# EasyVision-Ton/VMG

Measured on AMD Instinct MI355X. Metric: LR-frames/s (train: forward+loss+backward+AdamW), VMG-REDS-few_levels 4x SR, higher is better.
Workload: dtype bf16; 1 GPU; VMG-REDS-few_levels train step, per-GPU batch 4x7x3x64x64 -> 4x SR (BASELINE configs[1]); global_batch=4, frames_per_clip=7, parallelism=dp1, launch=eager, recompute_chains=False, fp8_chains=False

## Files before the change

include/vmg_hip.h:

```cpp
#ifndef VMG_HIP_H
#define VMG_HIP_H

#include <stdint.h>

#ifdef __cplusplus
extern "C" {
#endif

#define VMG_F32 0
#define VMG_BF16 1

#define VMG_ACT_NONE 0
#define VMG_ACT_RELU 1
#define VMG_ACT_LRELU 2
#define VMG_ACT_GELU 3

#define VMG_CONV_GENERAL 0
#define VMG_CONV_KSPLIT 2
#define VMG_CONV_WS 3
#define VMG_CONV_LINEAR_WRES 4
#define VMG_CONV_WSTAT 6

const char* vmg_last_error(void);
int vmg_version(void);
// ... 234 lines not shown
int64_t vmg_win3d_attn_bwd_ws_bytes(int B, int D, int H, int W, int heads, int wt);
int vmg_win3d_attn_bwd(int dtype, const void* q, const void* kv, const float* bq, const float* bkv, const float* table, const void* out,
                       const float* lse, const void* d_out, void* dq, void* dkv, float* dtable, float* dbq, float* dbkv, void* ws, int B, int D, int H, int W,
                       int C, int heads, int wt, int sd, int sh, int sw, void* stream);
int vmg_win3d_variant(int variant);

int vmg_maxpool_fwd(int dtype, const void* x, void* y, unsigned char* idx, int N, int H, int W, int C, int f, void* stream);
int vmg_maxpool_bwd(int dtype, const void* dy, const unsigned char* idx, void* dx, int N, int H, int W, int C, int f, void* stream);

int vmg_se_mlp_fwd(const float* m, const float* w1, const float* b1, const float* w2, const float* b2, float* pre, float* out, int G, int C,
                   int Hd, int Co, int act1, int mode, void* stream);
int vmg_se_mlp_bwd(const float* dout, const float* out, const float* m, const float* pre, const float* w1, const float* w2, float* dm,
                   float* dw1, float* db1, float* dw2, float* db2, float* ws, int G, int C, int Hd, int Co, int act1, int mode, float dm_scale,
                   int accumulate, void* stream);

int vmg_avgpool2_nhwc(int dtype, const void* x, void* y, int n, int h, int w, int c, void* stream);
int vmg_upsample2x_ac_fwd(const float* x, float* y, int n, int h, int w, int c, float scale, void* stream);
int vmg_upsample2x_ac_bwd(const float* dy, float* dx, int n, int h, int w, int c, float scale, void* stream);
int vmg_spy_operand_fwd(int dtype, const void* ref, const void* warped, const float* up, void* out, int64_t npix, void* stream);
int vmg_spy_operand_bwd(int dtype, const void* dx8, void* dwarped, float* dup, int64_t npix, void* stream);
int vmg_spy_flow_add(int dtype, const float* up, const void* res, float* out, int64_t n, void* stream);
int vmg_spy_prep(int dtype, const float* img, const float* mean, const float* stdv, void* out, int64_t n, int h, int w, void* stream);
typedef struct vmg_spy_module_desc {
  int N, H, W;
  const void* x;
  const void* packed[5];
  const float* bias[5];
  void* y[4];
  void* out;
  void* dpre[4];
// ... 95 lines not shown
```

vmg_amd/csrc/tab_ops.hip:

```cpp
#include "common.h"

namespace {

template <typename T>
struct V16 {
  static constexpr int N = 16 / sizeof(T);
  T v[N];
};

template <typename T, int VN>
__global__ __launch_bounds__(256) void group_reduce_kernel(const T* __restrict__ a, const T* __restrict__ b, const T* __restrict__ c3,
                                                           float* __restrict__ out, int G, long long R, int C, int mode, float scale,
                                                           int chunks) {
  struct alignas(sizeof(T) * VN) Vec { T v[VN]; };
  __shared__ float red[VN * 256];
  const int g = blockIdx.x / chunks, ck = blockIdx.x - g * chunks;
  const int tpr = C / VN;
  const int rpb = 256 / tpr;
  const int roff = threadIdx.x / tpr, cp = threadIdx.x - roff * tpr;
  const long long r0 = R * ck / chunks, r1 = R * (ck + 1) / chunks;
  float s[VN];
#pragma unroll
  for (int e = 0; e < VN; ++e) s[e] = 0.f;
  if (roff < rpb) {
// ... 492 lines not shown
  } else if (i < n1 + n2) {
    const int e = i - n1, o = e / Hd, j = e - o * Hd;
    for (int g = 0; g < G; ++g) s += dz2[(long long)g * Co + o] * se_act(pre[g * Hd + j], act1);
    dw2[e] = accumulate ? dw2[e] + s : s;
  } else if (i < n1 + n2 + Hd) {
    const int j = i - n1 - n2;
    for (int g = 0; g < G; ++g) s += dz1[g * Hd + j];
    db1[j] = accumulate ? db1[j] + s : s;
  } else if (i < n1 + n2 + Hd + Co) {
    const int o = i - n1 - n2 - Hd;
    for (int g = 0; g < G; ++g) s += dz2[(long long)g * Co + o];
    db2[o] = accumulate ? db2[o] + s : s;
  }
}

}

extern "C" int vmg_se_mlp_fwd(const float* m, const float* w1, const float* b1, const float* w2, const float* b2, float* pre, float* out, int G,
                              int C, int Hd, int Co, int act1, int mode, void* stream) {
  VMG_CHECK(m && w1 && w2 && pre && out && G > 0 && C > 0 && Hd > 0 && Co > 0, "se_mlp_fwd: bad arguments");
  VMG_CHECK((act1 == 1 || act1 == 3) && (mode == 0 || (mode == 1 && Co % 3 == 0)), "se_mlp_fwd: act1 is ReLU (1) or GELU (3); mode 1 needs Co = 3 * channels");
  VMG_CHECK((C + Hd) * 4 <= 64 * 1024, "se_mlp_fwd: C + Hd too large");
  hipLaunchKernelGGL(se_mlp_fwd_kernel, dim3(G), dim3(1024), (C + Hd) * 4, (hipStream_t)stream, m, w1, b1, w2, b2, pre, out, C, Hd, Co, act1, mode);
  VMG_LAUNCH_CHECK();
  return 0;
}

extern "C" int vmg_se_mlp_bwd(const float* dout, const float* out, const float* m, const float* pre, const float* w1, const float* w2, float* dm,
                              float* dw1, float* db1, float* dw2, float* db2, float* ws, int G, int C, int Hd, int Co, int act1, int mode,
                              float dm_scale, int accumulate, void* stream) {
// ... 84 lines not shown
  const int chunks = gr_chunks(G, R);
  VMG_CHECK((int64_t)G * chunks * C * 3 * (int64_t)sizeof(float) <= ws_bytes, "group_reduce3: workspace too small (vmg_group_reduce_ws_bytes)");
  hipStream_t st = (hipStream_t)stream;
  if (dtype == VMG_BF16)
    hipLaunchKernelGGL((group_reduce3_kernel<bf16, 8>), dim3(G * chunks), dim3(256), 0, st, (const bf16*)a, (const bf16*)b0, (const bf16*)b1,
                       (const bf16*)b2, ws, G, (long long)R, C, scale, chunks);
  else
    hipLaunchKernelGGL((group_reduce3_kernel<float, 4>), dim3(G * chunks), dim3(256), 0, st, (const float*)a, (const float*)b0, (const float*)b1,
                       (const float*)b2, ws, G, (long long)R, C, scale, chunks);
  VMG_LAUNCH_CHECK();
  hipLaunchKernelGGL(group_reduce_final_kernel, dim3(G * cdiv(3 * C, 16)), dim3(256), 0, st, (const float*)ws, out, G, chunks, 3 * C, scale);
  VMG_LAUNCH_CHECK();
  return 0;
}

extern "C" int vmg_tab_elementwise(int dtype, int op, const void* p0, const void* p1, const void* p2, const float* coef, const float* add,
                                   float s, void* o0, void* o1, void* o2, int64_t rows, int64_t R, int C, void* stream) {
  VMG_CHECK(dtype == VMG_F32 || dtype == VMG_BF16, "tab_elementwise: bad dtype");
  VMG_CHECK(op >= 0 && op <= 9 && p0 && o0 && rows > 0 && R > 0 && rows % R == 0 && C > 0, "tab_elementwise: bad arguments");
  const int vn = dtype == VMG_BF16 ? 8 : 4;
  VMG_CHECK(C % vn == 0, "tab_elementwise: C must be a multiple of %d", vn);
  static const unsigned char uses[10] = { 1 | 4,       4 | 8 | 16,  1 | 2 | 4,       4 | 8 | 16 | 32,
                                          1,         1 | 2 | 16,  4 | 8,         4,
                                          1 | 2 | 4,  1 | 2 | 4 | 16};
  const void* const ptrs[6] = {p1, p2, coef, add, o1, o2};
  static const char* const names[6] = {"p1", "p2", "coef", "add", "o1", "o2"};
  VMG_CHECK((((uintptr_t)p0 | (uintptr_t)o0) % 16) == 0, "tab_elementwise: pointers must be 16-byte aligned");
  for (int i = 0; i < 6; ++i) {
    const bool used = (uses[op] >> i) & 1;
    VMG_CHECK(!used || ptrs[i], "tab_elementwise: op %d needs %s", op, names[i]);
// ... 52 lines not shown
```

vmg_amd/functional.py:

```python
from __future__ import annotations

import contextlib
from typing import List, Optional, Sequence

import torch

from . import hip
from . import kernels as K
from .hip import HipError
from .wgrad import DEFERRED, _wgrad_entries, _wgrad_now, flush_deferred_wgrads, recorded, set_wgrad_mode

class _Fn(torch.autograd.Function):

    @classmethod
    def apply(cls, *args):
        return super(torch.autograd.Function, cls).apply(*args)


def _pad_to(n: int, m: int = 8) -> int:
    return (n + m - 1) // m * m


def choose_tiling(M: int, cout: int, ks: int, dtype: torch.dtype, src_ch: Optional[Sequence[int]] = None, pixel_shuffle: bool = False):
    if USE_WS and src_ch is not None and not pixel_shuffle:
# ... 10 lines not shown
        if cout == 288 and src_ch[0] == 144:
            return 5, 1, hip.CONV_LINEAR_WRES
        if cout == 144 and src_ch[0] == 288:
            return 3, 1, hip.CONV_LINEAR_WRES
    if dtype == torch.bfloat16 and ks == 3 and not pixel_shuffle and M >= (1 << 18) and src_ch is not None and len(src_ch) == 1 and \
            src_ch[0] <= 64 and src_ch[0] % 8 == 0 and cout in (16, 48, 64):
        return cout // 16, 1, hip.CONV_WSTAT
    if dtype == torch.bfloat16 and ks == 3 and not pixel_shuffle and M >= (1 << 20) and src_ch is not None and len(src_ch) == 1 and \
            (cout <= 16 or src_ch[0] <= 16):
        return None, 2, hip.CONV_GENERAL
    return None, 1, hip.CONV_GENERAL


USE_WS = True
GROUPED_DENSE = True

class _PlanState:

    def __init__(self):
        self.plan, self.stamp, self.wkey, self.ents, self.packs = K.PackPlan(), -1, None, [], []


def _from_param(ent) -> bool:
    pw, weight = ent[1], ent[2]
    return pw.call is not None and pw.call[0] == weight.data_ptr()


class _PackCache:

    def __init__(self):
# ... 817 lines not shown
        axis, chunk, Cp, shape = ctx.cfg
        return K.morph_tokens_gather(g.contiguous(), axis, chunk, Cp, Cp), None, None, None, None


def morph_linear(x: torch.Tensor, weight: torch.Tensor, bias: Optional[torch.Tensor], axis: str, chunk: int, Cp: int) -> torch.Tensor:
    if K.morph_fused_ok(x, chunk, Cp):
        return _MorphLinear.apply(x, weight, bias, axis, chunk, Cp)
    tok = _MorphGather.apply(x, axis, chunk, Cp)
    if tok.shape[-1] != Cp:
        padded, tok = tok, tok[:, :Cp]
        tok._vmg_padded = padded
    t = linear(tok, weight, bias, act=hip.ACT_RELU, alpha=1.0 / Cp)
    return _MorphScatter.apply(t, axis, chunk, Cp, tuple(x.shape))


class _ChannelAttention(_Fn):

    @staticmethod
    def forward(ctx, r, x, w1, b1, w2, b2, s):
        r, x = r.contiguous(), x.contiguous()
        N, C = r.shape[0], r.shape[-1]
        R = r.numel() // (N * C)
        m = K.group_reduce(r, N, scale=1.0 / R)
        pre, g = K.se_mlp_forward(m, w1.flatten(1), b1, w2.flatten(1), b2, hip.ACT_RELU, 0)
        out = K.tab_elementwise(K.OP_CA_FWD, r, x, coef=g, s=s, G=N)
        ctx.s, ctx.R = s, R
        ctx.save_for_backward(r, g, m, pre, w1, w2)
        DEFERRED.claim(ctx, w1, b1, w2, b2)
        return out

    @staticmethod
    def backward(ctx, dy):
        r, g, m, pre, w1, w2 = ctx.saved_tensors
        s, R = ctx.s, ctx.R
        dy = dy.contiguous()
        N = r.shape[0]
        dg = K.group_reduce(dy, N, b=r, mode=1, scale=s)
        dm, dw1, db1, dw2, db2 = K.se_mlp_backward(dg, g, m, pre, w1.flatten(1), w2.flatten(1), hip.ACT_RELU, 0, 1.0 / R, into=DEFERRED.into(ctx))
        d_r, d_x = K.tab_elementwise(K.OP_CA_BWD, dy, coef=g, add=dm, s=s, G=N, nout=2)
        DEFERRED.done(ctx)
        if ctx.direct:
            return d_r, d_x, None, None, None, None, None
        return (d_r, d_x, dw1.reshape(w1.shape), db1, dw2.reshape(w2.shape), db2, None)


def channel_attention_residual(r, x, w1, b1, w2, b2, out_scale: float):
    return _ChannelAttention.apply(r, x, w1, b1, w2, b2, float(out_scale))

class _ResidualDropPath(_Fn):

    @staticmethod
    def forward(ctx, res, y, g, gb=None):
        out = K.tab_elementwise(K.OP_CA_FWD, y.contiguous(), res.contiguous(), coef=g, s=1.0, G=g.shape[0])
# ... 66 lines not shown
            mask.div_(keep)
        g = (mask * scale).expand(B, C).contiguous()
    else:
        g = torch.full((B, C), float(scale), dtype=torch.float32, device=y.device)
    return _ResidualDropPath.apply(res, y, g)



class _ReweightMix(_Fn):

    @staticmethod
    def forward(ctx, h, w, c, fc1w, fc1b, fc2w, fc2b):
        h, w, c = h.contiguous(), w.contiguous(), c.contiguous()
        B, C = h.shape[0], h.shape[-1]
        R = h.numel() // (B * C)
        m = K.group_reduce(h, B, b=w, c3=c, scale=1.0 / R)
        pre, a = K.se_mlp_forward(m, fc1w, fc1b, fc2w, fc2b, hip.ACT_GELU, 1)
        y = K.tab_elementwise(K.OP_MIX_FWD, h, w, c, coef=a, G=B)
        ctx.R = R
        ctx.save_for_backward(h, w, c, a, m, pre, fc1w, fc2w)
        DEFERRED.claim(ctx, fc1w, fc1b, fc2w, fc2b)
        return y

    @staticmethod
    def backward(ctx, dy):
        h, w, c, a, m, pre, fc1w, fc2w = ctx.saved_tensors
        R = ctx.R
        dy = dy.contiguous()
        B, C = h.shape[0], h.shape[-1]
        da = K.group_reduce3(dy, h, w, c, B).reshape(B, 3 * C)
        dm, dw1, db1, dw2, db2 = K.se_mlp_backward(da, a, m, pre, fc1w, fc2w, hip.ACT_GELU, 1, 1.0 / R, into=DEFERRED.into(ctx))
        dh, dw, dc = K.tab_elementwise(K.OP_MIX_BWD, dy, coef=a, add=dm, G=B, nout=3)
        DEFERRED.done(ctx)
        if ctx.direct:
            return dh, dw, dc, None, None, None, None
        return dh, dw, dc, dw1, db1, dw2, db2


def reweight_mix(h, w, c, fc1w, fc1b, fc2w, fc2b):
    return _ReweightMix.apply(h, w, c, fc1w, fc1b, fc2w, fc2b)


class _ReweightMix2(_Fn):

    @staticmethod
    def forward(ctx, h, w, fc1w, fc1b, fc2w, fc2b):
# ... 599 lines not shown
```

vmg_amd/hip.py:

```python
from __future__ import annotations

import ctypes
import os
from ctypes import POINTER, c_char_p, c_float, c_int, c_int64, c_void_p

import torch

HERE = os.path.dirname(os.path.abspath(__file__))
LIB_PATH = os.environ.get("VMG_HIP_LIB") or os.path.join(HERE, "libvmg_hip.so")

F32, BF16 = 0, 1
ACT_NONE, ACT_RELU, ACT_LRELU, ACT_GELU = 0, 1, 2, 3
GATE_ACTS = {"tanh": 0, "sigmoid": 1, "relu": 2, "gelu": 3, "swish": 4}
SHIFT_VECTOR, SHIFT_ELEMENT = 1, 2
DWCONV_VECTOR, DWCONV_ELEMENT, DWCONV_PLAN_INTS = 1, 2, 8
CONV_GENERAL, CONV_KSPLIT, CONV_WS, CONV_LINEAR_WRES, CONV_WSTAT = 0, 2, 3, 4, 6
CONV_FAM_IGEMM, CONV_FAM_KSPLIT, CONV_FAM_WS, CONV_FAM_LINEAR_WRES, CONV_FAM_WSTAT = 1, 2, 3, 4, 5
CONV_PLAN_INTS = 11
MORPHFC_PLAN_INTS = 8
MORPH_ROUTE_ELEMENT, MORPH_ROUTE_LDS = 0, 1
WGRAD_V1, WGRAD_3, WGRAD_3B, WGRAD_L2, WGRAD_7 = 1, 2, 3, 4, 5


def wgrad_kernel_id(kind: int, a: int = 0, b: int = 0, c: int = 0) -> int:
# ... 104 lines not shown
    "vmg_win3d_variant": (c_int, [c_int]),
    "vmg_linear_wgrad2_multi": (c_int, [c_int, c_int, c_void_p, c_void_p, c_int64, c_int64, c_int, c_int64, c_int, c_void_p, c_int, c_int, c_int,
                                        c_void_p, c_void_p, c_void_p, c_int64, c_void_p]),
    "vmg_replay_build": (c_void_p, [c_void_p, c_void_p, c_void_p]),
    "vmg_replay_kernel_info": (c_int, [c_void_p, c_int, c_void_p, c_void_p, c_void_p, c_void_p]),
    "vmg_replay_run": (c_int, [c_void_p, c_int, c_int, c_void_p]),
    "vmg_replay_destroy": (None, [c_void_p]),
    "vmg_pack_entry_bytes": (c_int, []),
    "vmg_pack_entry": (c_int, [c_void_p, c_int, c_int, c_void_p, c_int, c_int, c_int, c_int, c_int, c_int, c_void_p, c_void_p, c_int, c_int, c_void_p,
                               c_int]),
    "vmg_pack_run": (c_int, [c_void_p, c_int, c_int, c_void_p]),
    "vmg_group_reduce3": (c_int, [c_int, c_void_p, c_void_p, c_void_p, c_void_p, c_void_p, c_int, c_int64, c_int, ctypes.c_float, c_void_p, c_int64, c_void_p]),
    "vmg_group_reduce_ws_bytes": (c_int64, []),
    "vmg_se_mlp_fwd": (c_int, [c_void_p] * 7 + [c_int] * 6 + [c_void_p]),
    "vmg_se_mlp_bwd": (c_int, [c_void_p] * 12 + [c_int] * 6 + [ctypes.c_float, c_int, c_void_p]),
    "vmg_maxpool_fwd": (c_int, [c_int, c_void_p, c_void_p, c_void_p, c_int, c_int, c_int, c_int, c_int, c_void_p]),
    "vmg_maxpool_bwd": (c_int, [c_int, c_void_p, c_void_p, c_void_p, c_int, c_int, c_int, c_int, c_int, c_void_p]),
    "vmg_avgpool2_nhwc": (c_int, [c_int, c_void_p, c_void_p, c_int, c_int, c_int, c_int, c_void_p]),
    "vmg_upsample2x_ac_fwd": (c_int, [c_void_p, c_void_p, c_int, c_int, c_int, c_int, c_float, c_void_p]),
    "vmg_upsample2x_ac_bwd": (c_int, [c_void_p, c_void_p, c_int, c_int, c_int, c_int, c_float, c_void_p]),
    "vmg_spy_operand_fwd": (c_int, [c_int, c_void_p, c_void_p, c_void_p, c_void_p, c_int64, c_void_p]),
    "vmg_spy_operand_bwd": (c_int, [c_int, c_void_p, c_void_p, c_void_p, c_int64, c_void_p]),
    "vmg_spy_flow_add": (c_int, [c_int, c_void_p, c_void_p, c_void_p, c_int64, c_void_p]),
    "vmg_spy_prep": (c_int, [c_int, c_void_p, c_void_p, c_void_p, c_void_p, c_int64, c_int, c_int, c_void_p]),
    "vmg_spy_module_fwd": (c_int, [POINTER(SpyModuleDesc), c_void_p]),
    "vmg_spy_module_bwd": (c_int, [POINTER(SpyModuleDesc), c_void_p]),
    "vmg_space_depth_ln_fwd": (c_int, [c_int, c_int, c_void_p, c_void_p, c_void_p, c_void_p, c_void_p, c_void_p, c_int, c_int, c_int, c_int, c_float, c_void_p]),
    "vmg_space_depth_ln_bwd": (c_int, [c_int, c_int, c_void_p, c_void_p, c_void_p, c_void_p, c_void_p, c_void_p, c_void_p, c_void_p, c_int, c_int, c_int, c_int,
                                       c_void_p, c_void_p]),
    "vmg_conv_wgrad_batched": (c_int, [c_int, c_int, c_int, POINTER(c_void_p), POINTER(c_void_p), c_int, c_int, c_int, c_int64, c_int,
# ... 154 lines not shown
```

vmg_amd/kernels.py:

```python
from __future__ import annotations

import collections
import ctypes
import os
import struct
from typing import Optional, Sequence, Tuple

import torch

from . import hip
from .hip import ConvDesc, HipError


def _intarr(v: Sequence[int]):
    return (ctypes.c_int * len(v))(*[int(x) for x in v])


def cout_tiles_for(cout: int, dtype: torch.dtype = torch.bfloat16, ks: int = 3) -> int:
    t = (cout + 15) // 16
    if t <= 1:
        return 1
    if ks == 7:
        return 2 if t == 2 else 4
    if t <= 4:
# ... 1299 lines not shown
        dm, ws = parts
        dw1, db1, dw2, db2 = into
        for t, n in zip(into, (Hd * C, Hd, Co * Hd, Co)):
            if t.dtype != torch.float32 or not t.is_contiguous() or t.numel() != n or not t.is_cuda:
                raise HipError("se_mlp: gradient buffers must be contiguous fp32 of the parameters' sizes")
    else:
        dm, ws, dw1, db1, dw2, db2 = parts
    hip.check(hip.lib().vmg_se_mlp_bwd(dout.data_ptr(), out.data_ptr(), m.data_ptr(), pre.data_ptr(), w1.data_ptr(), w2.data_ptr(), dm.data_ptr(),
                                       dw1.data_ptr(), db1.data_ptr(), dw2.data_ptr(), db2.data_ptr(), ws.data_ptr(), G, C, Hd, Co, act1, mode,
                                       float(dm_scale), 1 if into is not None else 0, hip.stream_ptr()), "vmg_se_mlp_bwd")
    if into is not None:
        return dm.view(G, C), dw1, db1, dw2, db2
    return dm.view(G, C), dw1.view(Hd, C), db1, dw2.view(Co, Hd), db2


SHIFT_ROUTES = {hip.SHIFT_VECTOR: "vector", hip.SHIFT_ELEMENT: "element"}


def patch_shift_route(Cs: int, dtype: torch.dtype, aligned: bool = True) -> str:
    r = hip.lib().vmg_patch_shift_plan(hip.dtype_code(dtype), int(Cs), int(bool(aligned)))
    if r not in SHIFT_ROUTES:
        raise HipError(f"patch_shift_route: no route for Cs = {Cs}, {dtype}")
    return SHIFT_ROUTES[r]


def _shift_args(who, x, others):
    hip.require_cuda(x, *others)
    if x.dim() != 4 or x.dtype not in (torch.float32, torch.bfloat16) or not x.is_contiguous():
        raise HipError(f"{who}: a contiguous fp32 / bf16 (N, H, W, Cs) tensor expected")
    if any(t.shape != x.shape or t.dtype != x.dtype or not t.is_contiguous() for t in others):
# ... 499 lines not shown
```

Baseline: 592.8 LR-frames/s.

## Fuse group pooling and SE gate MLP into single last-block-arrival kernels

New measurement: 587.1 LR-frames/s. About the same (-1.0%).

```diff
diff --git a/include/vmg_hip.h b/include/vmg_hip.h
--- a/include/vmg_hip.h
+++ b/include/vmg_hip.h
@@ -272,6 +272,15 @@
                    float* dw1, float* db1, float* dw2, float* db2, float* ws, int G, int C, int Hd, int Co, int act1, int mode, float dm_scale,
                    int accumulate, void* stream);
 
+int64_t vmg_pool_gate_ws_bytes(void);
+int vmg_pool_gate_fwd(int dtype, const void* a, const void* b, const void* c3, const float* w1, const float* b1, const float* w2, const float* b2,
+                      float* m, float* pre, float* out, int G, int64_t R, int C, int Hd, int Co, int act1, int mode, float scale, void* ws,
+                      int64_t ws_bytes, void* stream);
+int vmg_pool_gate_bwd(int dtype, int nb, const void* dy, const void* b0, const void* b1, const void* b2, const float* out, const float* m,
+                      const float* pre, const float* w1, const float* w2, float* dm, float* dw1, float* db1, float* dw2, float* db2, int G,
+                      int64_t R, int C, int Hd, int Co, int act1, int mode, float scale, float dm_scale, int accumulate, void* ws,
+                      int64_t ws_bytes, void* stream);
+
 int vmg_avgpool2_nhwc(int dtype, const void* x, void* y, int n, int h, int w, int c, void* stream);
 int vmg_upsample2x_ac_fwd(const float* x, float* y, int n, int h, int w, int c, float scale, void* stream);
 int vmg_upsample2x_ac_bwd(const float* dy, float* dx, int n, int h, int w, int c, float scale, void* stream);
diff --git a/vmg_amd/csrc/tab_ops.hip b/vmg_amd/csrc/tab_ops.hip
--- a/vmg_amd/csrc/tab_ops.hip
+++ b/vmg_amd/csrc/tab_ops.hip
@@ -530,6 +530,382 @@
   }
 }
 
+constexpr int PG_TREE = 16 * 65;
+constexpr int PG_MAXW = 3 * 512;
+constexpr int PG_MAXHD = 128;
+constexpr int PG_TAIL = PG_TREE + 2 * PG_MAXW + 2 * PG_MAXHD;
+constexpr int PG_PARAM_MAX = 12288;
+constexpr int PG_MAXG = 1024;
+
+__device__ __forceinline__ void pg_store(float* p, float v) { __hip_atomic_store(p, v, __ATOMIC_RELAXED, __HIP_MEMORY_SCOPE_AGENT); }
+__device__ __forceinline__ float pg_load(const float* p) { return __hip_atomic_load(p, __ATOMIC_RELAXED, __HIP_MEMORY_SCOPE_AGENT); }
+
+__device__ __forceinline__ bool pg_last_arrival(unsigned int* cnt, unsigned int n, unsigned int* tick) {
+  asm volatile("s_waitcnt vmcnt(0)" ::: "memory");
+  __syncthreads();
+  if (threadIdx.x == 0) {
+    const unsigned int t = __hip_atomic_fetch_add(cnt, 1u, __ATOMIC_RELAXED, __HIP_MEMORY_SCOPE_AGENT);
+    if (t == n - 1) __hip_atomic_exchange(cnt, 0u, __ATOMIC_RELAXED, __HIP_MEMORY_SCOPE_AGENT);
+    tick[0] = t;
+  }
+  __syncthreads();
+  return tick[0] == n - 1;
+}
+
+template <typename T, int VN>
+__device__ __forceinline__ void pg_pool1(const T* __restrict__ a, const T* __restrict__ b, const T* __restrict__ c3, float* part, float* red, int g,
+                                         int ck, long long R, int C, int mode, int chunks) {
+  struct alignas(sizeof(T) * VN) Vec { T v[VN]; };
+  const int tpr = C / VN;
+  const int rpb = 256 / tpr;
+  const int roff = threadIdx.x / tpr, cp = threadIdx.x - roff * tpr;
+  const long long r0 = R * ck / chunks, r1 = R * (ck + 1) / chunks;
+  float s[VN];
+#pragma unroll
+  for (int e = 0; e < VN; ++e) s[e] = 0.f;
+  if (roff < rpb) {
+    const long long base = (long long)g * R * C + VN * cp;
+    constexpr int U = 4;
+    for (long long r = r0 + roff; r < r1; r += (long long)U * rpb) {
+      Vec va[U], vb[U], vc[U];
+      bool ok[U];
+#pragma unroll
+      for (int u = 0; u < U; ++u) {
+        const long long rr = r + (long long)u * rpb;
+        ok[u] = rr < r1;
+        const long long o = base + (ok[u] ? rr : r) * C;
+        va[u] = *reinterpret_cast<const Vec*>(a + o);
+        if (b) vb[u] = *reinterpret_cast<const Vec*>(b + o);
+        if (c3) vc[u] = *reinterpret_cast<const Vec*>(c3 + o);
+      }
+#pragma unroll
+      for (int u = 0; u < U; ++u) {
+        if (!ok[u]) continue;
+        if (mode == 0) {
+          if (b && c3) {
+#pragma unroll
+            for (int e = 0; e < VN; ++e) s[e] += to_f32(va[u].v[e]) + to_f32(vb[u].v[e]) + to_f32(vc[u].v[e]);
+          } else if (b) {
+#pragma unroll
+            for (int e = 0; e < VN; ++e) s[e] += to_f32(va[u].v[e]) + to_f32(vb[u].v[e]);
+          } else {
+#pragma unroll
+            for (int e = 0; e < VN; ++e) s[e] += to_f32(va[u].v[e]);
+          }
+        } else {
+#pragma unroll
+          for (int e = 0; e < VN; ++e) s[e] += to_f32(va[u].v[e]) * to_f32(vb[u].v[e]);
+        }
+      }
+    }
+  }
+#pragma unroll
+  for (int e = 0; e < VN; ++e) red[e * 256 + threadIdx.x] = s[e];
+  __syncthreads();
+  for (int c = threadIdx.x; c < C; c += 256) {
+    const int cp2 = c / VN, e = c - cp2 * VN;
+    float t = 0.f;
+    for (int k = 0; k < rpb; ++k) t += red[e * 256 + k * tpr + cp2];
+    pg_store(part + ((long long)g * chunks + ck) * C + c, t);
+  }
+}
+
+template <typename T, int VN>
+__device__ __forceinline__ void pg_pool3(const T* __restrict__ a, const T* __restrict__ b0, const T* __restrict__ b1, const T* __restrict__ b2,
+                                         float* part, float* red, int g, int ck, long long R, int C, int chunks) {
+  struct alignas(sizeof(T) * VN) Vec { T v[VN]; };
+  const int tpr = C / VN;
+  const int rpb = 256 / tpr;
+  const int roff = threadIdx.x / tpr, cp = threadIdx.x - roff * tpr;
+  const long long r0 = R * ck / chunks, r1 = R * (ck + 1) / chunks;
+  float s[3][VN];
+#pragma unroll
+  for (int k = 0; k < 3; ++k)
+#pragma unroll
+    for (int e = 0; e < VN; ++e) s[k][e] = 0.f;
+  if (roff < rpb) {
+    const long long base = (long long)g * R * C + VN * cp;
+    for (long long r = r0 + roff; r < r1; r += rpb) {
+      const long long o = base + r * C;
+      const Vec va = *reinterpret_cast<const Vec*>(a + o);
+      const Vec v0 = *reinterpret_cast<const Vec*>(b0 + o), v1 = *reinterpret_cast<const Vec*>(b1 + o), v2 = *reinterpret_cast<const Vec*>(b2 + o);
+#pragma unroll
+      for (int e = 0; e < VN; ++e) {
+        const float d = to_f32(va.v[e]);
+        s[0][e] += d * to_f32(v0.v[e]);
+        s[1][e] += d * to_f32(v1.v[e]);
+        s[2][e] += d * to_f32(v2.v[e]);
+      }
+    }
+  }
+#pragma unroll
+  for (int k = 0; k < 3; ++k)
+#pragma unroll
+    for (int e = 0; e < VN; ++e) red[(k * VN + e) * 256 + threadIdx.x] = s[k][e];
+  __syncthreads();
+  for (int i = threadIdx.x; i < 3 * C; i += 256) {
+    const int c = i / 3, k = i - 3 * c;
+    const int cp2 = c / VN, e = c - cp2 * VN;
+    float t = 0.f;
+    for (int j = 0; j < rpb; ++j) t += red[(k * VN + e) * 256 + j * tpr + cp2];
+    pg_store(part + (((long long)g * chunks + ck) * C + c) * 3 + k, t);
+  }
+}
+
+__device__ __forceinline__ void pg_final_tree(const float* gpart, int chunks, int width, float scale, float* row, float* tree) {
+  const int q = threadIdx.x >> 4, cg = threadIdx.x & 15;
+  for (int c0 = 0; c0 < width; c0 += 64) {
+    float t[2][2] = {{0.f, 0.f}, {0.f, 0.f}};
+    for (int kb = 0; kb < chunks; kb += 256) {
+      unsigned long long v[2][16];
+#pragma unroll
+      for (int h = 0; h < 2; ++h) {
+        const int c = c0 + 32 * h + 2 * cg;
+#pragma unroll
+        for (int j = 0; j < 16; ++j) {
+          const int k = kb + q + 16 * j;
+          const unsigned int pair = ((unsigned int)k * (unsigned int)width + (unsigned int)c) >> 1;
+          v[h][j] = (c < width && k < chunks) ? __hip_atomic_load(reinterpret_cast<const unsigned long long*>(gpart) + pair, __ATOMIC_RELAXED,
+                                                                   __HIP_MEMORY_SCOPE_AGENT)
+                                              : 0ull;
+        }
+      }
+#pragma unroll
+      for (int h = 0; h < 2; ++h)
+#pragma unroll
+        for (int j = 0; j < 16; ++j)
+          if (kb + q + 16 * j < chunks) {
+            t[h][0] += __uint_as_float((unsigned int)v[h][j]);
+            t[h][1] += __uint_as_float((unsigned int)(v[h][j] >> 32));
+          }
+    }
+#pragma unroll
+    for (int h = 0; h < 2; ++h) {
+      tree[q * 65 + 32 * h + 2 * cg] = t[h][0];
+      tree[q * 65 + 32 * h + 2 * cg + 1] = t[h][1];
+    }
+    __syncthreads();
+    if (threadIdx.x < 64 && c0 + threadIdx.x < width) {
+      float u = 0.f;
+#pragma unroll
+      for (int i = 0; i < 16; ++i) u += tree[i * 65 + threadIdx.x];
+      row[c0 + threadIdx.x] = u * scale;
+    }
+    __syncthreads();
+  }
+}
+
+constexpr int PG_JB = 20;
+constexpr int PG_UJ = 9;
+
+__device__ __forceinline__ float pg_dot_hd(float s, const float* __restrict__ wr, int stride, const float* z, int Hd) {
+  for (int j0 = 0; j0 < Hd; j0 += PG_JB) {
+    float wv[PG_JB];
+#pragma unroll
+    for (int u = 0; u < PG_JB; ++u) wv[u] = wr[(long long)min(j0 + u, Hd - 1) * stride];
+#pragma unroll
+    for (int u = 0; u < PG_JB; ++u) s = j0 + u < Hd ? s + wv[u] * z[j0 + u] : s;
+  }
+  return s;
+}
+
+__device__ __forceinline__ void pg_stage(float* dst, const float* __restrict__ src, int n, bool vec4) {
+  constexpr int K = 8;
+  if (vec4) {
+    const int n4 = n >> 2;
+    for (int i0 = threadIdx.x; i0 < n4; i0 += 256 * K) {
+      float4 v[K];
+#pragma unroll
+      for (int k = 0; k < K; ++k) v[k] = reinterpret_cast<const float4*>(src)[min(i0 + 256 * k, n4 - 1)];
+#pragma unroll
+      for (int k = 0; k < K; ++k)
+        if (i0 + 256 * k < n4) reinterpret_cast<float4*>(dst)[i0 + 256 * k] = v[k];
+    }
+  } else {
+    for (int i0 = threadIdx.x; i0 < n; i0 += 256 * K) {
+      float v[K];
+#pragma unroll
+      for (int k = 0; k < K; ++k) v[k] = src[min(i0 + 256 * k, n - 1)];
+#pragma unroll
+      for (int k = 0; k < K; ++k)
+        if (i0 + 256 * k < n) dst[i0 + 256 * k] = v[k];
+    }
+  }
+}
+
+__device__ __forceinline__ void pg_mlp_fwd(const float* mrow, float* z1, float* lg, const float* sw1, const float* sb1, const float* w2s,
+                                           const float* __restrict__ w2g, const float* sb2, float* __restrict__ pre, float* __restrict__ out,
+                                           int g, int C, int Hd, int Co, int act1, int mode) {
+  const int tid = threadIdx.x, lane = tid & 63, wave = tid >> 6, nt = 256, nw = 4;
+  for (int j = wave; j < Hd; j += nw) {
+    float s = 0.f;
+    for (int c = lane; c < C; c += 64) s += sw1[j * C + c] * mrow[c];
+    s = wave_sum(s) + sb1[j];
+    if (lane == 0) { pre[(long long)g * Hd + j] = s; z1[j] = se_act(s, act1); }
+  }
+  __syncthreads();
+  for (int o = tid; o < Co; o += nt) {
+    float s;
+    if (w2s) s = pg_dot_hd(sb2[o], w2s + o * Hd, 1, z1, Hd);
+    else s = pg_dot_hd(sb2[o], w2g + (long long)o * Hd, 1, z1, Hd);
+    if (mode == 0) out[(long long)g * Co + o] = 1.f / (1.f + expf(-s));
+    else lg[o] = s;
+  }
+  if (mode == 0) return;
+  __syncthreads();
+  for (int c = tid; c < Co / 3; c += nt) {
+    const float z0 = lg[3 * c], z1_ = lg[3 * c + 1], z2 = lg[3 * c + 2];
+    const float mx = fmaxf(z0, fmaxf(z1_, z2));
+    const float e0 = expf(z0 - mx), e1 = expf(z1_ - mx), e2 = expf(z2 - mx), inv = 1.f / (e0 + e1 + e2);
+    float* orow = out + (long long)g * Co + 3 * c;
+    orow[0] = e0 * inv; orow[1] = e1 * inv; orow[2] = e2 * inv;
+  }
+}
+
+template <typename F>
+__device__ __forceinline__ void pg_param_sums(float* dst, int n, int accumulate, F sum) {
+  constexpr int K = 8;
+  for (int i0 = threadIdx.x; i0 < n; i0 += 256 * K) {
+    float old[K];
+#pragma unroll
+    for (int k = 0; k < K; ++k) old[k] = accumulate ? dst[min(i0 + 256 * k, n - 1)] : 0.f;
+#pragma unroll
+    for (int k = 0; k < K; ++k) {
+      const int i = i0 + 256 * k;
+      if (i < n) { const float t = sum(i); dst[i] = accumulate ? old[k] + t : t; }
+    }
+  }
+}
+
+template <typename T, int VN>
+__global__ __launch_bounds__(256, 4) void pool_gate_fwd_kernel(const T* __restrict__ a, const T* __restrict__ b, const T* __restrict__ c3,
+                                                            const float* __restrict__ w1, const float* __restrict__ b1,
+                                                            const float* __restrict__ w2, const float* __restrict__ b2, float* __restrict__ m,
+                                                            float* __restrict__ pre, float* __restrict__ out, float* part, unsigned int* cnt,
+                                                            long long R, int C, int Hd, int Co, int act1, int mode, float scale, int chunks,
+                                                            int stage_w2, int vec4) {
+  extern __shared__ __attribute__((aligned(16))) float dsm_raw[];
+  unsigned int* tick = reinterpret_cast<unsigned int*>(dsm_raw);
+  float* dsm = dsm_raw + 4;
+  const int g = blockIdx.x / chunks, ck = blockIdx.x - g * chunks;
+  pg_pool1<T, VN>(a, b, c3, part, dsm, g, ck, R, C, 0, chunks);
+  if (!pg_last_arrival(cnt + g, (unsigned int)chunks, tick)) return;
+  float* tree = dsm;
+  float* sw1 = tree + PG_TREE;
+  float* sw2 = sw1 + Hd * C;
+  float* mrow = sw2 + (stage_w2 ? Co * Hd : 0);
+  float* lg = mrow + C;
+  float* sb2 = lg + Co;
+  float* sb1 = sb2 + Co;
+  float* z1 = sb1 + Hd;
+  pg_stage(sw1, w1, Hd * C, vec4);
+  if (stage_w2) pg_stage(sw2, w2, Co * Hd, vec4);
+  for (int i = threadIdx.x; i < Co; i += 256) sb2[i] = b2 ? b2[i] : 0.f;
+  for (int i = threadIdx.x; i < Hd; i += 256) sb1[i] = b1 ? b1[i] : 0.f;
+  pg_final_tree(part + (long long)g * chunks * C, chunks, C, scale, mrow, tree);
+  for (int c = threadIdx.x; c < C; c += 256) m[(long long)g * C + c] = mrow[c];
+  pg_mlp_fwd(mrow, z1, lg, sw1, sb1, stage_w2 ? sw2 : nullptr, w2, sb2, pre, out, g, C, Hd, Co, act1, mode);
+}
+
+template <typename T, int VN, int NB>
+__global__ __launch_bounds__(256, 4) void pool_gate_bwd_kernel(const T* __restrict__ dy, const T* __restrict__ b0, const T* __restrict__ b1,
+                                                            const T* __restrict__ b2, const float* __restrict__ out,
+                                                            const float* __restrict__ m, const float* __restrict__ pre,
+                                                            const float* __restrict__ w1, const float* __restrict__ w2, float* __restrict__ dm,
+                                                            float* dw1, float* db1, float* dw2, float* db2, float* part, float* dzws,
+                                                            unsigned int* cnt, int G, long long R, int C, int Hd, int Co, int act1, int mode,
+                                                            float scale, float dm_scale, int accumulate, int chunks, int pmode) {
+  extern __shared__ __attribute__((aligned(16))) float dsm_raw[];
+  unsigned int* tick = reinterpret_cast<unsigned int*>(dsm_raw);
+  float* dsm = dsm_raw + 4;
+  const int g = blockIdx.x / chunks, ck = blockIdx.x - g * chunks;
+  if (NB == 1) pg_pool1<T, VN>(dy, b0, b1, part, dsm, g, ck, R, C, pmode, chunks);
+  else pg_pool3<T, VN>(dy, b0, b1, b2, part, dsm, g, ck, R, C, chunks);
+  if (!pg_last_arrival(cnt + g, (unsigned int)chunks, tick)) return;
+  const int tid = threadIdx.x, lane = tid & 63, wave = tid >> 6, nt = 256, nw = 4;
+  {
+    float* tree = dsm;
+    float* drow = dsm + PG_TREE;
+    float* dz2 = drow + PG_MAXW;
+    float* dz1 = dz2 + PG_MAXW;
+    float* prow = dz1 + PG_MAXHD;
+    for (int j = tid; j < Hd; j += nt) prow[j] = pre[(long long)g * Hd + j];
+    pg_final_tree(part + (long long)g * chunks * Co, chunks, Co, scale, drow, tree);
+    float* gz2 = dzws + (long long)g * Co;
+    float* gz1 = dzws + (long long)G * Co + (long long)g * Hd;
+    const float* orow = out + (long long)g * Co;
+    if (mode == 0) {
+      for (int o = tid; o < Co; o += nt) { const float v = drow[o] * orow[o] * (1.f - orow[o]); dz2[o] = v; pg_store(gz2 + o, v); }
+    } else {
+      for (int c = tid; c < Co / 3; c += nt) {
+        const float a0 = orow[3 * c], a1 = orow[3 * c + 1], a2 = orow[3 * c + 2];
+        const float d0 = drow[3 * c], d1 = drow[3 * c + 1], d2 = drow[3 * c + 2];
+        const float sd = a0 * d0 + a1 * d1 + a2 * d2;
+        const float v0 = a0 * (d0 - sd), v1 = a1 * (d1 - sd), v2 = a2 * (d2 - sd);
+        dz2[3 * c] = v0; dz2[3 * c + 1] = v1; dz2[3 * c + 2] = v2;
+        pg_store(gz2 + 3 * c, v0); pg_store(gz2 + 3 * c + 1, v1); pg_store(gz2 + 3 * c + 2, v2);
+      }
+    }
+    __syncthreads();
+    for (int jb = wave; jb < Hd; jb += nw * PG_UJ) {
+      float s[PG_UJ];
+#pragma unroll
+      for (int u = 0; u < PG_UJ; ++u) s[u] = 0.f;
+#pragma unroll 2
+      for (int o = lane; o < Co; o += 64) {
+        const float dv = dz2[o];
+        float wv[PG_UJ];
+#pragma unroll
+        for (int u = 0; u < PG_UJ; ++u) wv[u] = w2[(long long)o * Hd + min(jb + u * nw, Hd - 1)];
+#pragma unroll
+        for (int u = 0; u < PG_UJ; ++u) s[u] = jb + u * nw < Hd ? s[u] + dv * wv[u] : s[u];
+      }
+#pragma unroll
+      for (int u = 0; u < PG_UJ; ++u) {
+        const int j = jb + u * nw;
+        if (j < Hd) {
+          const float t = wave_sum(s[u]) * se_dact(prow[j], act1);
+          if (lane == 0) { dz1[j] = t; pg_store(gz1 + j, t); }
+        }
+      }
+    }
+    __syncthreads();
+    for (int c = tid; c < C; c += nt) dm[(long long)g * C + c] = pg_dot_hd(0.f, w1 + c, C, dz1, Hd) * dm_scale;
+  }
+  if (!pg_last_arrival(cnt + PG_MAXG, (unsigned int)G, tick)) return;
+  float* sz2 = dsm;
+  float* sz1 = sz2 + (long long)G * Co;
+  float* sm_ = sz1 + (long long)G * Hd;
+  float* sa = sm_ + (long long)G * C;
+  for (int i = tid; i < G * Co; i += nt) sz2[i] = pg_load(dzws + i);
+  for (int i = tid; i < G * Hd; i += nt) sz1[i] = pg_load(dzws + (long long)G * Co + i);
+  for (int i = tid; i < G * C; i += nt) sm_[i] = m[i];
+  for (int i = tid; i < G * Hd; i += nt) sa[i] = se_act(pre[i], act1);
+  __syncthreads();
+  pg_param_sums(dw1, Hd * C, accumulate, [&](int i) {
+    const int j = i / C, c = i - j * C;
+    float t = 0.f;
+    for (int gg = 0; gg < G; ++gg) t += sz1[gg * Hd + j] * sm_[gg * C + c];
+    return t;
+  });
+  pg_param_sums(dw2, Co * Hd, accumulate, [&](int e) {
+    const int o = e / Hd, j = e - o * Hd;
+    float t = 0.f;
+    for (int gg = 0; gg < G; ++gg) t += sz2[gg * Co + o] * sa[gg * Hd + j];
+    return t;
+  });
+  pg_param_sums(db1, Hd, accumulate, [&](int j) {
+    float t = 0.f;
+    for (int gg = 0; gg < G; ++gg) t += sz1[gg * Hd + j];
+    return t;
+  });
+  pg_param_sums(db2, Co, accumulate, [&](int o) {
+    float t = 0.f;
+    for (int gg = 0; gg < G; ++gg) t += sz2[gg * Co + o];
+    return t;
+  });
+}
+
 }
 
 extern "C" int vmg_se_mlp_fwd(const float* m, const float* w1, const float* b1, const float* w2, const float* b2, float* pre, float* out, int G,
@@ -644,6 +1020,94 @@
   return 0;
 }
 
+constexpr int64_t PG_PART = (int64_t)1024 * 3 * 512;
+constexpr int64_t PG_DZ = 16384;
+extern "C" int64_t vmg_pool_gate_ws_bytes() { return (PG_PART + PG_DZ) * (int64_t)sizeof(float) + (PG_MAXG + 4) * (int64_t)sizeof(unsigned int); }
+
+constexpr int PG_FWD_LDS = 8192;
+static int pg_fwd_tail(int C, int Hd, int Co, int stage_w2) { return PG_TREE + Hd * C + (stage_w2 ? Co * Hd : 0) + C + 2 * Co + 2 * Hd; }
+
+static int pg_common_checks(const char* who, int dtype, int G, int64_t R, int C, int Hd, int Co, int act1, int mode, const void* ws, int64_t ws_bytes) {
+  VMG_CHECK(dtype == VMG_F32 || dtype == VMG_BF16, "%s: bad dtype", who);
+  VMG_CHECK(G > 0 && G <= PG_MAXG && R > 0 && C > 0 && (C & 1) == 0 && C <= 512, "%s: bad arguments (G <= %d, C even, <= 512)", who, PG_MAXG);
+  VMG_CHECK(Hd > 0 && Hd <= PG_MAXHD && Co > 0 && Co <= PG_MAXW, "%s: Hd <= %d and Co <= %d expected", who, PG_MAXHD, PG_MAXW);
+  VMG_CHECK((act1 == 1 || act1 == 3) && (mode == 0 || (mode == 1 && Co % 3 == 0)), "%s: act1 is ReLU (1) or GELU (3); mode 1 needs Co = 3 * channels", who);
+  VMG_CHECK(ws && ((uintptr_t)ws % 16) == 0 && ws_bytes >= vmg_pool_gate_ws_bytes(), "%s: workspace missing, unaligned or too small (vmg_pool_gate_ws_bytes)", who);
+  return 0;
+}
+
+extern "C" int vmg_pool_gate_fwd(int dtype, const void* a, const void* b, const void* c3, const float* w1, const float* b1, const float* w2,
+                                 const float* b2, float* m, float* pre, float* out, int G, int64_t R, int C, int Hd, int Co, int act1, int mode,
+                                 float scale, void* ws, int64_t ws_bytes, void* stream) {
+  if (int rc = pg_common_checks("pool_gate_fwd", dtype, G, R, C, Hd, Co, act1, mode, ws, ws_bytes)) return rc;
+  VMG_CHECK(a && w1 && w2 && m && pre && out, "pool_gate_fwd: null pointer");
+  VMG_CHECK(b || !c3, "pool_gate_fwd: c3 needs b (the sum of two tensors is a + b)");
+  const int chunks = gr_chunks(G, R);
+  float* part = (float*)ws;
+  unsigned int* cnt = (unsigned int*)(part + PG_PART + PG_DZ);
+  hipStream_t st = (hipStream_t)stream;
+  const bool al16 = ((uintptr_t)a % 16 == 0) && (!b || (uintptr_t)b % 16 == 0) && (!c3 || (uintptr_t)c3 % 16 == 0);
+  const int stage_w2 = pg_fwd_tail(C, Hd, Co, 1) <= PG_FWD_LDS ? 1 : 0;
+  const int tail = pg_fwd_tail(C, Hd, Co, stage_w2);
+  VMG_CHECK(tail <= PG_FWD_LDS, "pool_gate_fwd: W1 (%d x %d) does not fit the finishing block's LDS stage", Hd, C);
+  const int vec4 = (((uintptr_t)w1 | (uintptr_t)w2) % 16 == 0 && (Hd * C) % 4 == 0 && (Co * Hd) % 4 == 0) ? 1 : 0;
+#define PG_FWD(T, VN)                                                                                                                             \
+  hipLaunchKernelGGL((pool_gate_fwd_kernel<T, VN>), dim3(G * chunks), dim3(256), sizeof(float) * (4 + (VN * 256 > tail ? VN * 256 : tail)), st,        \
+                     (const T*)a, (const T*)b, (const T*)c3, w1, b1, w2, b2, m, pre, out, part, cnt, (long long)R, C, Hd, Co, act1, mode, scale, \
+                     chunks, stage_w2, vec4)
+  if (dtype == VMG_BF16) {
+    if (C % 8 == 0 && al16) PG_FWD(bf16, 8);
+    else PG_FWD(bf16, 2);
+  } else {
+    if (C % 4 == 0 && al16) PG_FWD(float, 4);
+    else PG_FWD(float, 2);
+  }
+#undef PG_FWD
+  VMG_LAUNCH_CHECK();
+  return 0;
+}
+
+extern "C" int vmg_pool_gate_bwd(int dtype, int nb, const void* dy, const void* b0, const void* b1, const void* b2, const float* out, const float* m,
+                                 const float* pre, const float* w1, const float* w2, float* dm, float* dw1, float* db1, float* dw2, float* db2, int G,
+                                 int64_t R, int C, int Hd, int Co, int act1, int mode, float scale, float dm_scale, int accumulate, void* ws,
+                                 int64_t ws_bytes, void* stream) {
+  if (int rc = pg_common_checks("pool_gate_bwd", dtype, G, R, C, Hd, Co, act1, mode, ws, ws_bytes)) return rc;
+  VMG_CHECK((nb == 1 || nb == 3) && Co == nb * C, "pool_gate_bwd: nb is 1 or 3 and Co = nb * C");
+  VMG_CHECK(dy && b0 && (nb == 1 || (b1 && b2)) && out && m && pre && w1 && w2 && dm && dw1 && db1 && dw2 && db2, "pool_gate_bwd: null pointer");
+  const int64_t stage = (int64_t)G * (Co + 2 * Hd + C);
+  VMG_CHECK(stage <= PG_PARAM_MAX, "pool_gate_bwd: G * (Co + 2 Hd + C) = %lld floats exceed the parameter block's LDS stage (%d)", (long long)stage,
+            PG_PARAM_MAX);
+  const int chunks = gr_chunks(G, R);
+  float* part = (float*)ws;
+  float* dz = part + PG_PART;
+  unsigned int* cnt = (unsigned int*)(dz + PG_DZ);
+  hipStream_t st = (hipStream_t)stream;
+  auto lds = [&](int red) { int64_t f = red > PG_TAIL ? red : PG_TAIL; if (stage > f) f = stage; return (size_t)(f + 4) * sizeof(float); };
+#define PG_BWD(T, VN, NB)                                                                                                                       \
+  hipLaunchKernelGGL((pool_gate_bwd_kernel<T, VN, NB>), dim3(G * chunks), dim3(256), lds(NB * VN * 256), st, (const T*)dy, (const T*)b0,        \
+                     (const T*)b1, (const T*)b2, out, m, pre, w1, w2, dm, dw1, db1, dw2, db2, part, dz, cnt, G, (long long)R, C, Hd, Co, act1,  \
+                     mode, scale, dm_scale, accumulate, chunks, 1)
+  if (nb == 1) {
+    const bool al16 = ((uintptr_t)dy % 16 == 0) && ((uintptr_t)b0 % 16 == 0);
+    if (dtype == VMG_BF16) {
+      if (C % 8 == 0 && al16) PG_BWD(bf16, 8, 1);
+      else PG_BWD(bf16, 2, 1);
+    } else {
+      if (C % 4 == 0 && al16) PG_BWD(float, 4, 1);
+      else PG_BWD(float, 2, 1);
+    }
+  } else {
+    const int vn = dtype == VMG_BF16 ? 8 : 4;
+    VMG_CHECK(C % vn == 0 && C / vn <= 256, "pool_gate_bwd: three operands need C a multiple of %d", vn);
+    VMG_CHECK((((uintptr_t)dy | (uintptr_t)b0 | (uintptr_t)b1 | (uintptr_t)b2) % 16) == 0, "pool_gate_bwd: pointers must be 16-byte aligned");
+    if (dtype == VMG_BF16) PG_BWD(bf16, 8, 3);
+    else PG_BWD(float, 4, 3);
+  }
+#undef PG_BWD
+  VMG_LAUNCH_CHECK();
+  return 0;
+}
+
 extern "C" int vmg_tab_elementwise(int dtype, int op, const void* p0, const void* p1, const void* p2, const float* coef, const float* add,
                                    float s, void* o0, void* o1, void* o2, int64_t rows, int64_t R, int C, void* stream) {
   VMG_CHECK(dtype == VMG_F32 || dtype == VMG_BF16, "tab_elementwise: bad dtype");
diff --git a/vmg_amd/functional.py b/vmg_amd/functional.py
--- a/vmg_amd/functional.py
+++ b/vmg_amd/functional.py
@@ -48,6 +48,7 @@
 
 USE_WS = True
 GROUPED_DENSE = True
+POOL_GATE_FUSED = False
 
 class _PlanState:
 
@@ -895,6 +896,10 @@
     return _MorphScatter.apply(t, axis, chunk, Cp, tuple(x.shape))
 
 
+def _pool_gate_fused(x, G, C, Hd, Co) -> bool:
+    return POOL_GATE_FUSED and K.pool_gate_ok(G, C, Hd, Co) and K.pool_gate_workspace(x.device) is not None
+
+
 class _ChannelAttention(_Fn):
 
     @staticmethod
@@ -902,8 +907,11 @@
         r, x = r.contiguous(), x.contiguous()
         N, C = r.shape[0], r.shape[-1]
         R = r.numel() // (N * C)
-        m = K.group_reduce(r, N, scale=1.0 / R)
-        pre, g = K.se_mlp_forward(m, w1.flatten(1), b1, w2.flatten(1), b2, hip.ACT_RELU, 0)
+        if _pool_gate_fused(r, N, C, w1.shape[0], w2.shape[0]):
+            m, pre, g = K.pool_gate_forward(r, N, w1.flatten(1), b1, w2.flatten(1), b2, hip.ACT_RELU, 0, 1.0 / R)
+        else:
+            m = K.group_reduce(r, N, scale=1.0 / R)
+            pre, g = K.se_mlp_forward(m, w1.flatten(1), b1, w2.flatten(1), b2, hip.ACT_RELU, 0)
         out = K.tab_elementwise(K.OP_CA_FWD, r, x, coef=g, s=s, G=N)
         ctx.s, ctx.R = s, R
         ctx.save_for_backward(r, g, m, pre, w1, w2)
@@ -916,8 +924,11 @@
         s, R = ctx.s, ctx.R
         dy = dy.contiguous()
         N = r.shape[0]
-        dg = K.group_reduce(dy, N, b=r, mode=1, scale=s)
-        dm, dw1, db1, dw2, db2 = K.se_mlp_backward(dg, g, m, pre, w1.flatten(1), w2.flatten(1), hip.ACT_RELU, 0, 1.0 / R, into=DEFERRED.into(ctx))
+        if _pool_gate_fused(dy, N, r.shape[-1], w1.shape[0], w2.shape[0]):
+            dm, dw1, db1, dw2, db2 = K.pool_gate_backward(dy, (r,), N, g, m, pre, w1.flatten(1), w2.flatten(1), hip.ACT_RELU, 0, s, 1.0 / R, into=DEFERRED.into(ctx))
+        else:
+            dg = K.group_reduce(dy, N, b=r, mode=1, scale=s)
+            dm, dw1, db1, dw2, db2 = K.se_mlp_backward(dg, g, m, pre, w1.flatten(1), w2.flatten(1), hip.ACT_RELU, 0, 1.0 / R, into=DEFERRED.into(ctx))
         d_r, d_x = K.tab_elementwise(K.OP_CA_BWD, dy, coef=g, add=dm, s=s, G=N, nout=2)
         DEFERRED.done(ctx)
         if ctx.direct:
@@ -1014,8 +1025,11 @@
         h, w, c = h.contiguous(), w.contiguous(), c.contiguous()
         B, C = h.shape[0], h.shape[-1]
         R = h.numel() // (B * C)
-        m = K.group_reduce(h, B, b=w, c3=c, scale=1.0 / R)
-        pre, a = K.se_mlp_forward(m, fc1w, fc1b, fc2w, fc2b, hip.ACT_GELU, 1)
+        if _pool_gate_fused(h, B, C, fc1w.shape[0], fc2w.shape[0]):
+            m, pre, a = K.pool_gate_forward(h, B, fc1w, fc1b, fc2w, fc2b, hip.ACT_GELU, 1, 1.0 / R, b=w, c3=c)
+        else:
+            m = K.group_reduce(h, B, b=w, c3=c, scale=1.0 / R)
+            pre, a = K.se_mlp_forward(m, fc1w, fc1b, fc2w, fc2b, hip.ACT_GELU, 1)
         y = K.tab_elementwise(K.OP_MIX_FWD, h, w, c, coef=a, G=B)
         ctx.R = R
         ctx.save_for_backward(h, w, c, a, m, pre, fc1w, fc2w)
@@ -1028,8 +1042,11 @@
         R = ctx.R
         dy = dy.contiguous()
         B, C = h.shape[0], h.shape[-1]
-        da = K.group_reduce3(dy, h, w, c, B).reshape(B, 3 * C)
-        dm, dw1, db1, dw2, db2 = K.se_mlp_backward(da, a, m, pre, fc1w, fc2w, hip.ACT_GELU, 1, 1.0 / R, into=DEFERRED.into(ctx))
+        if _pool_gate_fused(dy, B, C, fc1w.shape[0], fc2w.shape[0]) and C % (8 if dy.dtype == torch.bfloat16 else 4) == 0:
+            dm, dw1, db1, dw2, db2 = K.pool_gate_backward(dy, (h, w, c), B, a, m, pre, fc1w, fc2w, hip.ACT_GELU, 1, 1.0, 1.0 / R, into=DEFERRED.into(ctx))
+        else:
+            da = K.group_reduce3(dy, h, w, c, B).reshape(B, 3 * C)
+            dm, dw1, db1, dw2, db2 = K.se_mlp_backward(da, a, m, pre, fc1w, fc2w, hip.ACT_GELU, 1, 1.0 / R, into=DEFERRED.into(ctx))
         dh, dw, dc = K.tab_elementwise(K.OP_MIX_BWD, dy, coef=a, add=dm, G=B, nout=3)
         DEFERRED.done(ctx)
         if ctx.direct:
diff --git a/vmg_amd/hip.py b/vmg_amd/hip.py
--- a/vmg_amd/hip.py
+++ b/vmg_amd/hip.py
@@ -142,6 +142,10 @@
     "vmg_group_reduce_ws_bytes": (c_int64, []),
     "vmg_se_mlp_fwd": (c_int, [c_void_p] * 7 + [c_int] * 6 + [c_void_p]),
     "vmg_se_mlp_bwd": (c_int, [c_void_p] * 12 + [c_int] * 6 + [ctypes.c_float, c_int, c_void_p]),
+    "vmg_pool_gate_ws_bytes": (c_int64, []),
+    "vmg_pool_gate_fwd": (c_int, [c_int] + [c_void_p] * 10 + [c_int, c_int64] + [c_int] * 5 + [ctypes.c_float, c_void_p, c_int64, c_void_p]),
+    "vmg_pool_gate_bwd": (c_int, [c_int, c_int] + [c_void_p] * 14 + [c_int, c_int64] + [c_int] * 5 + [ctypes.c_float, ctypes.c_float, c_int, c_void_p,
+                                                                                                    c_int64, c_void_p]),
     "vmg_maxpool_fwd": (c_int, [c_int, c_void_p, c_void_p, c_void_p, c_int, c_int, c_int, c_int, c_int, c_void_p]),
     "vmg_maxpool_bwd": (c_int, [c_int, c_void_p, c_void_p, c_void_p, c_int, c_int, c_int, c_int, c_int, c_void_p]),
     "vmg_avgpool2_nhwc": (c_int, [c_int, c_void_p, c_void_p, c_int, c_int, c_int, c_int, c_void_p]),
diff --git a/vmg_amd/kernels.py b/vmg_amd/kernels.py
--- a/vmg_amd/kernels.py
+++ b/vmg_amd/kernels.py
@@ -1337,6 +1337,99 @@
     return dm.view(G, C), dw1.view(Hd, C), db1, dw2.view(Co, Hd), db2
 
 
+POOL_GATE_MAX_HD, POOL_GATE_MAX_STAGE = 128, 12288
+POOL_GATE_SPARES = 2
+
+
+def pool_gate_workspace(device) -> Optional[torch.Tensor]:
+    key = ("vmg_pool_gate_ws_bytes", device, hip.stream_ptr())
+    ws = _WS.get(key)
+    if ws is None:
+        spares = _WS.setdefault(("vmg_pool_gate_spares", device), None)
+        if not torch.cuda.is_current_stream_capturing():
+            make = lambda: torch.zeros(int(hip.lib().vmg_pool_gate_ws_bytes()), dtype=torch.uint8, device=device)
+            if spares is None:
+                _WS["vmg_pool_gate_spares", device] = [make() for _ in range(POOL_GATE_SPARES)]
+            ws = _WS[key] = make()
+        elif spares:
+            ws = _WS[key] = spares.pop()
+    return ws
+
+
+def pool_gate_ok(G: int, C: int, Hd: int, Co: int) -> bool:
+    return (G <= 1024 and C % 2 == 0 and C <= 512 and Hd <= POOL_GATE_MAX_HD and G * (Co + 2 * Hd + C) <= POOL_GATE_MAX_STAGE
+            and 1040 + Hd * C + C + 2 * Co + 2 * Hd <= 8192)
+
+
+def pool_gate_forward(a: torch.Tensor, G: int, w1: torch.Tensor, b1, w2: torch.Tensor, b2, act1: int, mode: int, scale: float,
+                      b: Optional[torch.Tensor] = None, c3: Optional[torch.Tensor] = None, ws: Optional[torch.Tensor] = None):
+    hip.require_cuda(a, b, c3, w1, w2)
+    C = a.shape[-1]
+    rows = a.numel() // C
+    if rows % G or not a.is_contiguous() or any(t is not None and (t.shape != a.shape or t.dtype != a.dtype or not t.is_contiguous()) for t in (b, c3)):
+        raise HipError("pool_gate_forward: contiguous tensors of one shape / dtype covering G groups expected")
+    Hd, Co = w1.shape[0], w2.shape[0]
+    for t in (w1, w2, b1, b2):
+        if t is not None and (t.dtype != torch.float32 or not t.is_contiguous()):
+            raise HipError("pool_gate_forward: contiguous fp32 parameters only")
+    if w1.shape != (Hd, C) or w2.shape != (Co, Hd):
+        raise HipError(f"pool_gate_forward: W1 ({Hd}, {C}) and W2 ({Co}, {Hd}) expected")
+    ws = pool_gate_workspace(a.device) if ws is None else ws
+    if ws is None:
+        raise HipError("pool_gate_forward: no workspace (create it outside graph capture)")
+    buf = torch.empty(G * (C + Hd), dtype=torch.float32, device=a.device)
+    m, pre = buf[:G * C].view(G, C), buf[G * C:].view(G, Hd)
+    out = torch.empty(G, Co, dtype=torch.float32, device=a.device)
+    ptr = lambda t: t.data_ptr() if t is not None else None
+    hip.check(hip.lib().vmg_pool_gate_fwd(hip.dtype_code(a.dtype), a.data_ptr(), ptr(b), ptr(c3), w1.data_ptr(), ptr(b1), w2.data_ptr(), ptr(b2),
+                                          m.data_ptr(), pre.data_ptr(), out.data_ptr(), G, rows // G, C, Hd, Co, act1, mode, float(scale),
+                                          ws.data_ptr(), ws.numel(), hip.stream_ptr()), "vmg_pool_gate_fwd")
+    return m, pre, out
+
+
+def pool_gate_backward(dy: torch.Tensor, bs, G: int, out: torch.Tensor, m: torch.Tensor, pre: torch.Tensor, w1: torch.Tensor, w2: torch.Tensor,
+                       act1: int, mode: int, scale: float, dm_scale: float, into=None, ws: Optional[torch.Tensor] = None):
+    hip.require_cuda(dy, *bs, out, m, pre, w1, w2)
+    if len(bs) not in (1, 3):
+        raise HipError("pool_gate_backward: one or three multiplicands")
+    C = dy.shape[-1]
+    rows = dy.numel() // C
+    if rows % G or any(t.shape != dy.shape or t.dtype != dy.dtype or not t.is_contiguous() for t in (dy, *bs)):
+        raise HipError("pool_gate_backward: contiguous tensors of one shape / dtype covering G groups expected")
+    Hd, Co = w1.shape[0], w2.shape[0]
+    for t in (out, m, pre, w1, w2):
+        if t.dtype != torch.float32 or not t.is_contiguous():
+            raise HipError("pool_gate_backward: contiguous fp32 tensors only")
+    if m.shape != (G, C) or pre.shape != (G, Hd) or out.numel() != G * Co or Co != len(bs) * C or w1.shape != (Hd, C) or w2.shape != (Co, Hd):
+        raise HipError("pool_gate_backward: m (G, C), pre (G, Hd), out (G, Co), W1 (Hd, C), W2 (Co, Hd) with Co = C per multiplicand expected")
+    ws = pool_gate_workspace(dy.device) if ws is None else ws
+    if ws is None:
+        raise HipError("pool_gate_backward: no workspace (create it outside graph capture)")
+    sizes = (G * C,) if into is not None else (G * C, Hd * C, Hd, Co * Hd, Co)
+    buf = torch.empty(sum(sizes), dtype=torch.float32, device=dy.device)
+    parts, o = [], 0
+    for n in sizes:
+        parts.append(buf[o:o + n])
+        o += n
+    if into is not None:
+        (dm,) = parts
+        dw1, db1, dw2, db2 = into
+        for t, n in zip(into, (Hd * C, Hd, Co * Hd, Co)):
+            if t.dtype != torch.float32 or not t.is_contiguous() or t.numel() != n or not t.is_cuda:
+                raise HipError("pool_gate_backward: gradient buffers must be contiguous fp32 of the parameters' sizes")
+    else:
+        dm, dw1, db1, dw2, db2 = parts
+    b = list(bs) + [None] * (3 - len(bs))
+    ptr = lambda t: t.data_ptr() if t is not None else None
+    hip.check(hip.lib().vmg_pool_gate_bwd(hip.dtype_code(dy.dtype), len(bs), dy.data_ptr(), ptr(b[0]), ptr(b[1]), ptr(b[2]), out.data_ptr(),
+                                          m.data_ptr(), pre.data_ptr(), w1.data_ptr(), w2.data_ptr(), dm.data_ptr(), dw1.data_ptr(), db1.data_ptr(),
+                                          dw2.data_ptr(), db2.data_ptr(), G, rows // G, C, Hd, Co, act1, mode, float(scale), float(dm_scale),
+                                          1 if into is not None else 0, ws.data_ptr(), ws.numel(), hip.stream_ptr()), "vmg_pool_gate_bwd")
+    if into is not None:
+        return dm.view(G, C), dw1, db1, dw2, db2
+    return dm.view(G, C), dw1.view(Hd, C), db1, dw2.view(Co, Hd), db2
+
+
 SHIFT_ROUTES = {hip.SHIFT_VECTOR: "vector", hip.SHIFT_ELEMENT: "element"}
 
 
```
